# ElijahHyndman/PAPTeam_OpticalFlow

Measured on AMD Instinct MI355X. Metric: Mpix/s per frame-pair (fixed SOR iters) at 1920x1080; max-abs d(u,v) vs ref, higher is better.
Workload: dtype f64

## Files before the change

papteam_opticalflow_amd/csrc/kernels.hip:

```cpp
#include "common.h"
#include "sampler.h"

#include <cmath>

namespace papof {

namespace {

constexpr int BX = 64, BY = 4;

inline dim3 grid2d(int W, int H, int planes = 1) { return dim3((W + BX - 1) / BX, (H + BY - 1) / BY, planes); }
inline Rect region(const Rect* rc, int W, int H) { return rc ? *rc : Rect{0, 0, W, H}; }
inline dim3 grid2d(const Rect& r, int planes = 1) { return grid2d(r.x1 - r.x0, r.y1 - r.y0, planes); }

__device__ __forceinline__ void stamp_now(unsigned long long* s) {
    if (s && (blockIdx.x | blockIdx.y | blockIdx.z | threadIdx.x | threadIdx.y) == 0u) *s = __builtin_amdgcn_s_memrealtime();
}
__global__ void k_stamp(unsigned long long* s) { stamp_now(s); }

__device__ __forceinline__ int clampi(int x, int n) {
    x = x < 0 ? 0 : x;
    return x > n - 1 ? n - 1 : x;
}

__device__ __forceinline__ bool xcd_tile(int ntx, int nty, int& tx, int& ty) {
    const int ntiles = ntx * nty, per = (ntiles + 7) >> 3;
    const int vt = (int)(blockIdx.x & 7u) * per + (int)(blockIdx.x >> 3);
    if ((int)(blockIdx.x >> 3) >= per || vt >= ntiles) return false;
    ty = vt / ntx;
    tx = vt - ty * ntx;
    return true;
}
static inline unsigned xcd_grid(int ntx, int nty) { return 8u * (unsigned)(((size_t)ntx * nty + 7) / 8); }

__global__ void k_hwc_to_planar(const double* __restrict__ hwc, double* __restrict__ planar, int H, int W, int C) {
    const int j = blockIdx.x * BX + threadIdx.x, i = blockIdx.y * BY + threadIdx.y;
    if (j >= W || i >= H) return;
    const size_t o = (size_t)i * W + j, np = (size_t)H * W;
    hwc += blockIdx.z * np * C;
    planar += blockIdx.z * np * C;
    for (int k = 0; k < C; k++) planar[k * np + o] = hwc[o * C + k];
}

__global__ void k_hwc_u8_to_planar(const unsigned char* __restrict__ hwc, double* __restrict__ planar, int H, int W,
                                   int C) {
    const int j = blockIdx.x * BX + threadIdx.x, i = blockIdx.y * BY + threadIdx.y;
    if (j >= W || i >= H) return;
    const size_t o = (size_t)i * W + j, np = (size_t)H * W;
    hwc += blockIdx.z * np * C;
    planar += blockIdx.z * np * C;
    for (int k = 0; k < C; k++) planar[k * np + o] = (double)hwc[o * C + k] / 255.0;
}

__global__ void k_planar_to_hwc(const double* __restrict__ planar, double* __restrict__ hwc, int H, int W, int C) {
    const int j = blockIdx.x * BX + threadIdx.x, i = blockIdx.y * BY + threadIdx.y;
    if (j >= W || i >= H) return;
    const size_t o = (size_t)i * W + j, np = (size_t)H * W;
    for (int k = 0; k < C; k++) hwc[o * C + k] = planar[k * np + o];
}

__device__ __forceinline__ double tensor_load(const void* p, int dtype, long long o) {
    if (dtype == PAPOF_DTYPE_U8) return (double)static_cast<const unsigned char*>(p)[o] / 255.0;
    if (dtype == PAPOF_DTYPE_F32) return (double)static_cast<const float*>(p)[o];
    return static_cast<const double*>(p)[o];
}

__global__ __launch_bounds__(256) void k_ingest_frames(const papof_tensor a, const papof_tensor b, int pairs,
                                                       double* __restrict__ planar, long long H, long long W, long long C,
                                                       long long total) {
    const long long i = (long long)blockIdx.x * blockDim.x + threadIdx.x;
    if (i >= total) return;
    const long long np = H * W, f = i / (np * C), r = i - f * np * C, c = r / np, px = r - c * np, row = px / W,
                    col = px - row * W;
    const bool second = pairs && (f & 1);
    const long long fi = pairs ? f >> 1 : f;
    const long long o = fi * (second ? b.stride[0] : a.stride[0]) + row * (second ? b.stride[1] : a.stride[1]) +
                        col * (second ? b.stride[2] : a.stride[2]) + c * (second ? b.stride[3] : a.stride[3]);
    planar[i] = tensor_load(second ? b.data : a.data, second ? b.dtype : a.dtype, o);
}

constexpr double kInitMax = 1e6;
__device__ __forceinline__ bool init_refused(double x) { return !(fabs(x) <= kInitMax); }

__global__ __launch_bounds__(256) void k_init_check(const papof_tensor t, long long H, long long W, long long total,
                                                    unsigned* __restrict__ flag) {
    const long long i = (long long)blockIdx.x * blockDim.x + threadIdx.x;
    if (i >= total) return;
    const long long np = H * W, p = i / (np * 2), r = i - p * np * 2, c = r / np, px = r - c * np, row = px / W,
                    col = px - row * W;
    const long long o = p * t.stride[0] + row * t.stride[1] + col * t.stride[2] + c * t.stride[3];
    if (init_refused(tensor_load(t.data, t.dtype, o))) atomicOr(flag, 1u);
}

__global__ __launch_bounds__(256) void k_init_sanitize(double* __restrict__ planar, long long total) {
    const long long i = (long long)blockIdx.x * blockDim.x + threadIdx.x;
    if (i >= total) return;
    if (init_refused(planar[i])) planar[i] = 0.0;
}

__global__ __launch_bounds__(256) void k_emit_outputs(const double* __restrict__ src, const papof_tensor dst, int comp_major,
                                                      long long H, long long W, long long K, long long total) {
    const long long i = (long long)blockIdx.x * blockDim.x + threadIdx.x;
    if (i >= total) return;
    const long long np = H * W, p = i / (np * K), r = i - p * np * K;
    const long long k = comp_major ? r / np : r % K, px = comp_major ? r - k * np : r / K, row = px / W, col = px - row * W;
    const long long o = p * dst.stride[0] + row * dst.stride[1] + col * dst.stride[2] + k * dst.stride[3];
    const double v = src[i];
    if (dst.dtype == PAPOF_DTYPE_F32)
        static_cast<float*>(dst.data)[o] = (float)v;
    else
        static_cast<double*>(dst.data)[o] = v;
}

constexpr int kFbTX = 64, kFbTY = 4;
__global__ __launch_bounds__(kFbTX * kFbTY) void k_fb_check(const papof_tensor fw, const papof_tensor bw, const papof_tensor mask,
                                                         int H, int W, double a1, double a2) {
    const int tx = (W + kFbTX - 1) / kFbTX;
    const int x = (int)(blockIdx.x % tx) * kFbTX + threadIdx.x, r = (int)(blockIdx.x / tx) * kFbTY + threadIdx.y;
    if (x >= W || r >= H) return;
    const long long p = blockIdx.y >> 1;
    const int dir = blockIdx.y & 1;
    const papof_tensor& f = dir ? bw : fw;
    const papof_tensor& b = dir ? fw : bw;
    const long long of = p * f.stride[0] + r * f.stride[1] + x * f.stride[2];
    const double u = load_flow(f, of), v = load_flow(f, of + f.stride[3]);
    const double X = (double)x + u, Y = (double)r + v;
    bool occluded = true;
    if (X >= 0 && X <= (double)(W - 1) && Y >= 0 && Y <= (double)(H - 1)) {
        double bu, bv;
        sample_flow(b, p * b.stride[0], taps_at(X, Y, H, W), bu, bv);
        occluded = !fb_passes(u, v, bu, bv, a1, a2);
    }
    static_cast<unsigned char*>(mask.data)[p * mask.stride[0] + r * mask.stride[1] + x * mask.stride[2] + dir * mask.stride[3]] =
        occluded ? 1 : 0;
}

__global__ void k_filter_h(const double* __restrict__ src, double* __restrict__ dst, int H, int W, Taps f, Rect rc) {
    const int j = rc.x0 + blockIdx.x * BX + threadIdx.x, i = rc.y0 + blockIdx.y * BY + threadIdx.y;
    if (j >= rc.x1 || i >= rc.y1) return;
    const size_t np = (size_t)H * W;
    const double* row = src + blockIdx.z * np + (size_t)i * W;
    double acc = 0.0;
    for (int l = -f.fsize; l <= f.fsize; l++) acc += row[clampi(j + l, W)] * f.t[l + f.fsize];
    dst[blockIdx.z * np + (size_t)i * W + j] = acc;
}

__global__ void k_filter_v(const double* __restrict__ src, double* __restrict__ dst, int H, int W, Taps f, Rect rc) {
    const int j = rc.x0 + blockIdx.x * BX + threadIdx.x, i = rc.y0 + blockIdx.y * BY + threadIdx.y;
    if (j >= rc.x1 || i >= rc.y1) return;
    const size_t np = (size_t)H * W;
    const double* p = src + blockIdx.z * np + j;
    double acc = 0.0;
    for (int l = -f.fsize; l <= f.fsize; l++) acc += p[(size_t)clampi(i + l, H) * W] * f.t[l + f.fsize];
    dst[blockIdx.z * np + (size_t)i * W + j] = acc;
}

// ... 622 lines not shown
        } else if (I.lap != nullptr && I.lap[k] < 1E-20) {
            psi = 0.0;
        } else {
            psi = 1 / (2 * sqrt(t + 0.001 * 0.001));
        }
        const double pgx = psi * gx, pgy = psi * gy;
        if (planes == 1) {
            sxy = pgx * gy;
            sx2 = pgx * gx;
            sy2 = pgy * gy;
            stx = pgx * gt;
            sty = pgy * gt;
        } else {
            sxy += pgx * gy;
            sx2 += pgx * gx;
            sy2 += pgy * gy;
            stx += pgx * gt;
            sty += pgy * gt;
        }
    };
    if (PLANES > 0) {
#pragma unroll
        for (int k = 0; k < PLANES; k++) channel(k);
    } else {
#pragma unroll 1
        for (int k = 0; k < planes; k++) channel(k);
    }
    if (planes > 1) {
        sxy = sxy / planes;
        sx2 = sx2 / planes;
        sy2 = sy2 / planes;
        stx = stx / planes;
        sty = sty / planes;
    }
    SystemCell c;
    if (EDGE) {
        c.b1 = -stx - alpha * laplacian_at(u, phi, i, j, H, W);
        c.b2 = -sty - alpha * laplacian_at(v, phi, i, j, H, W);
        sor_diagonals(phi, i, j, H, W, sx2, sy2, alpha, omega, c.a1, c.a2);
    } else {
        const double pc = phi[o], pl = phi[o - 1], pu = phi[o - W];
        const double uc = u[o], vc = v[o];
        double lu = 0.0, lv = 0.0;
        lu -= (u[o + 1] - uc) * pc;
        lu += (uc - u[o - 1]) * pl;
        lu -= (u[o + W] - uc) * pc;
        lu += (uc - u[o - W]) * pu;
        lv -= (v[o + 1] - vc) * pc;
        lv += (vc - v[o - 1]) * pl;
        lv -= (v[o + W] - vc) * pc;
        lv += (vc - v[o - W]) * pu;
        c.b1 = -stx - alpha * lu;
        c.b2 = -sty - alpha * lv;
        double coeff = 0.0;
        coeff += pl;
        coeff += pc;
        coeff += pu;
        coeff += pc;
        coeff *= alpha;
        c.a1 = omega / (sx2 + alpha * 0.05 + coeff);
        c.a2 = omega / (sy2 + alpha * 0.05 + coeff);
    }
    c.phi = phi[o];
    c.xy = sxy;
    c.x2 = sx2;
    c.y2 = sy2;
    return c;
}

__global__ void k_assemble(const double* __restrict__ blend, const double* __restrict__ imdt,
                           const double* __restrict__ phi, const double* __restrict__ u,
                           const double* __restrict__ v, int H, int W, int planes, double alpha, double omega,
                           double* __restrict__ o_phi, double* __restrict__ o_xy, double* __restrict__ o_a1,
                           double* __restrict__ o_a2, double* __restrict__ o_b1, double* __restrict__ o_b2,
                           double* __restrict__ o_x2, double* __restrict__ o_y2, Taps d, Increment I, Rect rc,
                           unsigned long long* stamp) {
    stamp_now(stamp);
    const int j = rc.x0 + blockIdx.x * BX + threadIdx.x, i = rc.y0 + blockIdx.y * BY + threadIdx.y;
    if (j >= rc.x1 || i >= rc.y1) return;
    const size_t o = (size_t)i * W + j;
    const SystemCell c = assemble_cell(blend, imdt, phi, u, v, i, j, H, W, planes, alpha, omega, d, I);
    o_phi[o] = c.phi;
    o_xy[o] = c.xy;
    o_a1[o] = c.a1;
    o_a2[o] = c.a2;
    o_b1[o] = c.b1;
    o_b2[o] = c.b2;
    if (o_x2) o_x2[o] = c.x2;
    if (o_y2) o_y2[o] = c.y2;
}

#ifndef PAPOF_V_ASMCOLS
#define PAPOF_V_ASMCOLS 16
#endif
constexpr int kTileJ = PAPOF_V_ASMCOLS;
#ifndef PAPOF_V_ASMROWS
#define PAPOF_V_ASMROWS 16
#endif
constexpr int kAsmRows = PAPOF_V_ASMROWS;
struct double2s {
    double x, y;
};
template <int PLANES, bool FAST>
__global__ __launch_bounds__(256) void k_assemble_skew(const double* __restrict__ blend,
                                                       const double* __restrict__ imdt,
                                                       const double* __restrict__ phi, const double* __restrict__ u,
                                                       const double* __restrict__ v, int H, int W, int planes,
                                                       double alpha, double omega, SkewIdx sk,
                                                       double2s* __restrict__ pa, double2s* __restrict__ pb,
                                                       double2s* __restrict__ pc, double* __restrict__ o_x2,
                                                       double* __restrict__ o_y2, Taps d, Increment I,
                                                       unsigned long long* stamp, int row0, int row1) {
    __shared__ double stage[6][kAsmRows][kTileJ + 1];
    stamp_now(stamp);
    const int ib = row0 + blockIdx.y * kAsmRows, j0 = blockIdx.x * kTileJ, tid = threadIdx.x;
    const bool interior = ib >= 2 && ib + kAsmRows + 2 <= H && j0 >= 2 && j0 + kTileJ + 2 <= W;
    for (int c = tid; c < kAsmRows * kTileJ; c += 256) {
        const int r = c / kTileJ, jj = c - r * kTileJ;
        const int i = ib + r, j = j0 + jj;
        if (i < row1 && j < W) {
            const SystemCell s =
                interior ? assemble_cell<false, PLANES, FAST>(blend, imdt, phi, u, v, i, j, H, W, planes, alpha, omega, d, I)
                         : assemble_cell<true, PLANES, FAST>(blend, imdt, phi, u, v, i, j, H, W, planes, alpha, omega, d, I);
            stage[0][r][jj] = s.phi;
            stage[1][r][jj] = s.xy;
            stage[2][r][jj] = s.a1;
            stage[3][r][jj] = s.a2;
            stage[4][r][jj] = s.b1;
            stage[5][r][jj] = s.b2;
            if (o_x2) o_x2[(size_t)i * W + j] = s.x2;
            if (o_y2) o_y2[(size_t)i * W + j] = s.y2;
        }
    }
    __syncthreads();
    const int g = tid / kTileJ, jj = tid - g * kTileJ;
    const int j = j0 + jj;
    if (j >= W) return;
    for (int pp = g; pp <= kAsmRows + kTileJ - 2; pp += 256 / kTileJ) {
        const int r = pp - jj;
        if (r < 0 || r >= kAsmRows) continue;
        const int i = ib + r;
        if (i >= row1) continue;
        const size_t q = skew_cell(i, j, sk);
        pa[q] = double2s{stage[0][r][jj], stage[1][r][jj]};
        pb[q] = double2s{stage[2][r][jj], stage[3][r][jj]};
        pc[q] = double2s{stage[4][r][jj], stage[5][r][jj]};
    }
}

constexpr int kFT = 16, kFH = 4, kFW = kFT + 2 * kFH;
struct SixPlanes {
    double* q[6];
};
template <int PLANES, bool SKEW, bool BATCH = false>
__global__ __launch_bounds__(256, 1) void k_flow_system(const double* __restrict__ im1, const double* __restrict__ im2,
                                                     const double* __restrict__ u, const double* __restrict__ v,
                                                     const double* __restrict__ im1s, int H, int W, double alpha,
                                                     double omega, SkewIdx sk, SixPlanes out, Taps g, Taps d,
                                                     unsigned long long* stamp, unsigned* __restrict__ wit, double wit_thr,
                                                     unsigned mark, int row0, int row1, BatchK bk) {
    if (BATCH) {
        const size_t p = blockIdx.y;
        im1s += batch_frames(bk, p, im1, im2);
        u += p * bk.uv;
        v += p * bk.uv;
        if (wit != nullptr) wit += p * bk.wit;
#pragma unroll
        for (int q = 0; q < 6; q++) out.q[q] += p * bk.sp;
    }
    constexpr int NT = kFT * kFT, HWc = kFT + 2 * kFH;
    __shared__ double raw[kFW][HWc + 1];
    __shared__ double hs[kFW][kFT + 4 + 1];
    __shared__ double bl[kFT + 4][kFT + 4 + 1];
    __shared__ double it[kFT][kFT + 1];
    __shared__ double ph[kFT + 1][kFT + 1 + 1];
    __shared__ double stage[6][kFT][kFT + 1];
    stamp_now(stamp);
    const int ntx = (W + kFT - 1) / kFT, ntiles = ntx * ((row1 - row0 + kFT - 1) / kFT), per = (ntiles + 7) >> 3;
    const int vt = (int)(blockIdx.x & 7u) * per + (int)(blockIdx.x >> 3);
    if ((int)(blockIdx.x >> 3) >= per || vt >= ntiles) return;
    const int tby = vt / ntx, tbx = vt - tby * ntx;
    const int ib = row0 + tby * kFT, j0 = tbx * kFT, tid = threadIdx.x;
    const size_t np = (size_t)H * W;
    const int vy0 = max(0, row0 - kFH), vy1 = min(H, row1 + kFH);
    const bool interior = ib >= vy0 + kFH && ib + kFT <= row1 && ib + kFT + kFH <= vy1 && j0 >= kFH && j0 + kFT + kFH <= W;
    constexpr int kPer = (kFW * HWc + NT - 1) / NT;
    int t_o[kPer], t_x0[kPer], t_y0[kPer];
    double t_dx[kPer], t_dy[kPer];
    bool t_in[kPer], t_out[kPer];
#pragma unroll
    for (int q = 0; q < kPer; q++) {
        const int c = tid + q * NT, r = c / HWc, cc = c - r * HWc;
        const int i = ib - kFH + r, j = j0 - kFH + cc;
        t_in[q] = c < kFW * HWc && i >= vy0 && i < vy1 && j >= 0 && j < W;
        t_o[q] = t_in[q] ? i * W + j : 0;
        double x = 0.0, y = 0.0;
        t_out[q] = false;
        if (t_in[q]) {
            y = i + v[t_o[q]];
            x = j + u[t_o[q]];
            t_out[q] = x < 0 || x > W - 1 || y < 0 || y > H - 1;
            if (t_out[q]) {
                x = j;
                y = i;
            }
        }
        t_x0[q] = (int)x;
        t_y0[q] = (int)y;
        t_dx[q] = x - t_x0[q];
        t_dy[q] = y - t_y0[q];
    }
    for (int c = tid; c < (kFT + 1) * (kFT + 1); c += NT) {
        const int r = c / (kFT + 1), cc = c - r * (kFT + 1);
        const int i = ib - 1 + r, j = j0 - 1 + cc;
        if (i < 0 || i >= min(H, row1) || j < 0 || j >= W) continue;
        const size_t o = (size_t)i * W + j;
        const double uc = u[o], vc = v[o];
        double ur = 0.0, vr = 0.0, ud = 0.0, vd = 0.0;
        if (j < W - 1) {
            ur = u[o + 1];
            vr = v[o + 1];
        }
        if (i < H - 1) {
            ud = u[o + W];
            vd = v[o + W];
        }
        const double ux = j < W - 1 ? ur - uc : 0.0;
        const double uy = i < H - 1 ? ud - uc : 0.0;
        const double vx = j < W - 1 ? vr - vc : 0.0;
        const double vy = i < H - 1 ? vd - vc : 0.0;
        const double tt = ux * ux + uy * uy + vx * vx + vy * vy;
        ph[r][cc] = 0.5 / sqrt(tt + 0.001 * 0.001);
    }
    const int orow = tid / kFT, ocol = tid - orow * kFT;
    const int oi = ib + orow, oj = j0 + ocol;
    const bool own = oi < row1 && oj < W;
    double sxy = 0.0, sx2 = 0.0, sy2 = 0.0, stx = 0.0, sty = 0.0;
    const bool sampler = wit != nullptr && tid < 64 &&
                         (ntiles <= 256 || ((tbx + 5 * tby) & 15) == 0);
    constexpr int kP3 = ((kFT + 4) * (kFT + 4) + NT - 1) / NT;
    double gv[kPer][4], s1v[kP3], wv = 0.0;
    const auto load_gathers = [&](int k) {
        const double *p1 = im1 + k * np, *p2 = im2 + k * np;
#pragma unroll
        for (int q = 0; q < kPer; q++) {
            const double* src = t_out[q] ? p1 : p2;
            const int x0 = t_x0[q], y0 = t_y0[q], x1 = min(x0 + 1, W - 1), y1 = min(y0 + 1, H - 1);
            gv[q][0] = src[y0 * W + x0];
            gv[q][1] = src[y1 * W + x0];
            gv[q][2] = src[y0 * W + x1];
            gv[q][3] = src[y1 * W + x1];
        }
        if (sampler) wv = p1[t_o[0]];
    };
    const auto load_s1 = [&](int k) {
        const double* ps = im1s + k * np;
#pragma unroll
        for (int q = 0; q < kP3; q++) {
            const int c = min(tid + q * NT, (kFT + 4) * (kFT + 4) - 1), r = c / (kFT + 4), cc = c - r * (kFT + 4);
            s1v[q] = ps[(size_t)clampi(ib - 2 + r, H) * W + clampi(j0 - 2 + cc, W)];
        }
    };
    load_gathers(0);
    load_s1(0);
#pragma unroll 1
    for (int k = 0; k < PLANES; k++) {
        bool hit = false;
#pragma unroll
        for (int q = 0; q < kPer; q++) {
            const int c = tid + q * NT, r = c / HWc, cc = c - r * HWc;
            const double dx = t_dx[q], dy = t_dy[q], ex = 1.0 - dx, ey = 1.0 - dy;
            double res = 0.0;
            res += gv[q][0] * (ex * ey);
            res += gv[q][1] * (ex * dy);
            res += gv[q][2] * (dx * ey);
            res += gv[q][3] * (dx * dy);
            res = t_out[q] ? gv[q][0] : res;
            if (t_in[q]) raw[r][cc] = res;
            if (sampler && q == 0) {
                const double dd = fabs(wv - res);
                hit = t_in[q] && dd >= wit_thr && dd < 1000000;
            }
        }
        if (sampler) {
            const unsigned long long hits = __ballot(hit);
            if (hits != 0ull && tid == 0) wit[k] = mark;
        }
        if (k + 1 < PLANES) load_gathers(k + 1);
        __syncthreads();
        if (interior) {
            for (int c = tid; c < kFW * (kFT + 4); c += NT) {
                const int r = c / (kFT + 4), cc = c - r * (kFT + 4);
                double acc = 0.0;
#pragma unroll
                for (int l = -2; l <= 2; l++) acc += raw[r][cc + 2 + l] * g.t[l + 2];
                hs[r][cc] = acc;
            }
        } else {
            for (int c = tid; c < kFW * (kFT + 4); c += NT) {
                const int r = c / (kFT + 4), cc = c - r * (kFT + 4);
                const int i = ib - kFH + r, j = j0 - 2 + cc;
                if (i < 0 || i >= H || j < 0 || j >= W) continue;
                double acc = 0.0;
#pragma unroll
                for (int l = -2; l <= 2; l++) acc += raw[r][clampi(j + l, W) - (j0 - kFH)] * g.t[l + 2];
                hs[r][cc] = acc;
            }
        }
        __syncthreads();
#pragma unroll
        for (int q = 0; q < kP3; q++) {
            const int c = tid + q * NT, r = c / (kFT + 4), cc = c - r * (kFT + 4);
            const int i = ib - 2 + r, j = j0 - 2 + cc;
            if (c >= (kFT + 4) * (kFT + 4) || i < 0 || i >= H || j < 0 || j >= W) continue;
            double s2 = 0.0;
            if (interior) {
#pragma unroll
                for (int l = -2; l <= 2; l++) s2 += hs[r + 2 + l][cc] * g.t[l + 2];
            } else {
#pragma unroll
                for (int l = -2; l <= 2; l++) s2 += hs[clampi(i + l, H) - (ib - kFH)][cc] * g.t[l + 2];
            }
            const double s1 = s1v[q];
            double t = s1;
            t *= 0.4;
            t += s2 * 0.6;
            bl[r][cc] = t;
            if (r >= 2 && r < kFT + 2 && cc >= 2 && cc < kFT + 2) it[r - 2][cc - 2] = s2 - s1;
        }
        if (k + 1 < PLANES) load_s1(k + 1);
        __syncthreads();
        if (own) {
            double gx = 0.0, gy = 0.0;
            if (interior) {
#pragma unroll
                for (int l = -2; l <= 2; l++) gx += bl[orow + 2][ocol + 2 + l] * d.t[l + 2];
#pragma unroll
                for (int l = -2; l <= 2; l++) gy += bl[orow + 2 + l][ocol + 2] * d.t[l + 2];
            } else {
#pragma unroll
                for (int l = -2; l <= 2; l++) gx += bl[orow + 2][clampi(oj + l, W) - (j0 - 2)] * d.t[l + 2];
#pragma unroll
                for (int l = -2; l <= 2; l++) gy += bl[clampi(oi + l, H) - (ib - 2)][ocol + 2] * d.t[l + 2];
            }
            const double gt = it[orow][ocol];
            double t = gt;
            t *= t;
            const double psi = 1 / (2 * sqrt(t + 0.001 * 0.001));
            const double pgx = psi * gx, pgy = psi * gy;
            if (PLANES == 1) {
                sxy = pgx * gy;
                sx2 = pgx * gx;
                sy2 = pgy * gy;
                stx = pgx * gt;
                sty = pgy * gt;
            } else {
                sxy += pgx * gy;
                sx2 += pgx * gx;
                sy2 += pgy * gy;
                stx += pgx * gt;
                sty += pgy * gt;
            }
        }
    }
    if (own) {
        if (PLANES > 1) {
            sxy = sxy / PLANES;
            sx2 = sx2 / PLANES;
            sy2 = sy2 / PLANES;
            stx = stx / PLANES;
            sty = sty / PLANES;
        }
        const int i = oi, j = oj;
        const size_t o = (size_t)i * W + j;
        const double pc_ = ph[orow + 1][ocol + 1];
        const double pl = j > 0 ? ph[orow + 1][ocol] : 0.0, pu = i > 0 ? ph[orow][ocol + 1] : 0.0;
        const double uc = u[o], vc = v[o];
        double lu = 0.0, lv = 0.0;
        if (j < W - 1) {
            lu -= (u[o + 1] - uc) * pc_;
            if (j > 0) lu += (uc - u[o - 1]) * pl;
        }
        if (i < H - 1) {
            lu -= (u[o + W] - uc) * pc_;
            if (i > 0) lu += (uc - u[o - W]) * pu;
        }
        if (j < W - 1) {
            lv -= (v[o + 1] - vc) * pc_;
            if (j > 0) lv += (vc - v[o - 1]) * pl;
        }
        if (i < H - 1) {
            lv -= (v[o + W] - vc) * pc_;
            if (i > 0) lv += (vc - v[o - W]) * pu;
        }
        double coeff = 0.0;
        if (j > 0) coeff += pl;
        if (j < W - 1) coeff += pc_;
        if (i > 0) coeff += pu;
        if (i < H - 1) coeff += pc_;
        coeff *= alpha;
        const double a1 = omega / (sx2 + alpha * 0.05 + coeff), a2 = omega / (sy2 + alpha * 0.05 + coeff);
        const double b1 = -stx - alpha * lu, b2 = -sty - alpha * lv;
        if (SKEW) {
            stage[0][orow][ocol] = pc_;
            stage[1][orow][ocol] = sxy;
            stage[2][orow][ocol] = a1;
            stage[3][orow][ocol] = a2;
            stage[4][orow][ocol] = b1;
            stage[5][orow][ocol] = b2;
        } else {
            out.q[0][o] = pc_;
            out.q[1][o] = sxy;
            out.q[2][o] = a1;
            out.q[3][o] = a2;
            out.q[4][o] = b1;
            out.q[5][o] = b2;
        }
    }
    if (!SKEW) return;
    double2s* const pa = reinterpret_cast<double2s*>(out.q[0]);
    double2s* const pb = reinterpret_cast<double2s*>(out.q[2]);
    double2s* const pc = reinterpret_cast<double2s*>(out.q[4]);
    __syncthreads();
    const int grp = tid / kFT, jj = tid - grp * kFT, j = j0 + jj;
    if (j >= W) return;
    for (int pp = grp; pp <= 2 * kFT - 2; pp += kFT) {
        const int r = pp - jj;
        if (r < 0 || r >= kFT) continue;
        const int i = ib + r;
        if (i >= row1) continue;
        const size_t q = skew_cell(i, j, sk);
        pa[q] = double2s{stage[0][r][jj], stage[1][r][jj]};
        pb[q] = double2s{stage[2][r][jj], stage[3][r][jj]};
        pc[q] = double2s{stage[4][r][jj], stage[5][r][jj]};
    }
}

template <bool SKEW>
__global__ void k_sor_prep(const double* __restrict__ phi, const double* __restrict__ imdxy,
                           const double* __restrict__ imdx2, const double* __restrict__ imdy2,
                           const double* __restrict__ rhs1, const double* __restrict__ rhs2, int H, int W,
                           double alpha, double omega, SkewIdx sk, double* __restrict__ o_phi,
                           double* __restrict__ o_xy, double* __restrict__ o_a1, double* __restrict__ o_a2,
                           double* __restrict__ o_b1, double* __restrict__ o_b2) {
    const int j = blockIdx.x * BX + threadIdx.x, i = blockIdx.y * BY + threadIdx.y;
    if (j >= W || i >= H) return;
    const size_t o = (size_t)i * W + j;
    double a1, a2;
    sor_diagonals(phi, i, j, H, W, imdx2[o], imdy2[o], alpha, omega, a1, a2);
    const size_t q = sor_index<SKEW>(i, j, W, sk);
    o_phi[q] = phi[o];
    o_xy[q] = imdxy[o];
    o_a1[q] = a1;
    o_a2[q] = a2;
    o_b1[q] = rhs1[o];
    o_b2[q] = rhs2[o];
}

template <bool SKEW>
__global__ void k_sor_unpack(const double* __restrict__ sdu, const double* __restrict__ sdv,
                             double* __restrict__ du, double* __restrict__ dv, int H, int W, SkewIdx sk) {
    const int j = blockIdx.x * BX + threadIdx.x, i = blockIdx.y * BY + threadIdx.y;
    if (j >= W || i >= H) return;
    const size_t o = (size_t)i * W + j;
    if (SKEW) {
        const size_t q = 2 * dudv_cell(i, j, sk);
        du[o] = sdu[q];
        dv[o] = sdu[q + 1];
    } else {
        du[o] = sdu[o];
        dv[o] = sdv[o];
    }
}

__global__ void k_update_warp(const double* __restrict__ sdu, const double* __restrict__ sdv, double* __restrict__ u,
                              double* __restrict__ v, const double* __restrict__ im1,
                              const double* __restrict__ im2, double* __restrict__ warp, int H, int W, int planes, Rect rc,
                              int do_warp, unsigned long long* stamp) {
    stamp_now(stamp);
    const int j = rc.x0 + blockIdx.x * BX + threadIdx.x, i = rc.y0 + blockIdx.y * BY + threadIdx.y;
    if (j >= rc.x1 || i >= rc.y1) return;
// ... 414 lines not shown
}

int filter_hv(papof_handle* h, const double* src, double* dst, double* tmp, int H, int W, int planes, const Taps& fh,
              const Taps& fv) {
    if (fh.fsize > kHvMaxF || fv.fsize > kHvMaxF) {
        if (!tmp) return PAPOF_EINVAL;
        PAPOF_TRY(filter_h(h, src, tmp, H, W, planes, fh));
        return filter_v(h, tmp, dst, H, W, planes, fv);
    }
    const dim3 grid((W + BX - 1) / BX, (H + kHvRows - 1) / kHvRows, planes), block(BX, BY);
    const int f = fh.fsize == fv.fsize ? fh.fsize : -1;
    if (PAPOF_V_HVSTAGED && f >= 1 && f <= 3) {
        const dim3 sgrid(xcd_grid((W + BX - 1) / BX, (H + kHvsRows - 1) / kHvsRows), 1, planes);
        if (f == 1)
            hipLaunchKernelGGL(k_filter_hv_staged<1>, sgrid, block, 0, h->stream, src, dst, H, W, fh, fv);
        else if (f == 2)
            hipLaunchKernelGGL(k_filter_hv_staged<2>, sgrid, block, 0, h->stream, src, dst, H, W, fh, fv);
        else
            hipLaunchKernelGGL(k_filter_hv_staged<3>, sgrid, block, 0, h->stream, src, dst, H, W, fh, fv);
        LAUNCH_CHECK();
        return PAPOF_OK;
    }
    if (f == 1)
        hipLaunchKernelGGL(k_filter_hv<1>, grid, block, 0, h->stream, src, dst, H, W, fh, fv);
    else if (f == 2)
        hipLaunchKernelGGL(k_filter_hv<2>, grid, block, 0, h->stream, src, dst, H, W, fh, fv);
    else if (f == 3)
        hipLaunchKernelGGL(k_filter_hv<3>, grid, block, 0, h->stream, src, dst, H, W, fh, fv);
    else
        hipLaunchKernelGGL(k_filter_hv<-1>, grid, block, 0, h->stream, src, dst, H, W, fh, fv);
    LAUNCH_CHECK();
    return PAPOF_OK;
}

int resize(papof_handle* h, const double* src, double* dst, int sh, int sw, int planes, int dh, int dw, double xr,
           double yr, bool use_post, double post, const Rect* rc) {
    const Rect r = region(rc, dw, dh);
    if (r.empty()) return PAPOF_OK;
    hipLaunchKernelGGL(k_resize, dim3(xcd_grid((r.x1 - r.x0 + BX - 1) / BX, (r.y1 - r.y0 + BY - 1) / BY), 1, planes), dim3(BX, BY), 0, h->stream, src, dst, sh, sw, dh, dw, xr, yr,
                       use_post ? 1 : 0, post, r, take_stamp(h));
    LAUNCH_CHECK();
    return PAPOF_OK;
}

int im2feature(papof_handle* h, const double* im, double* feat, int H, int W, int C, unsigned* nz, int frames, size_t nz_stride) {
    const size_t np = (size_t)H * W;
    if (C == 3) {
        hipLaunchKernelGGL((frames > 1 ? k_im2feature_tiled<3, true> : k_im2feature_tiled<3, false>), dim3(xcd_grid((W + BX - 1) / BX, (H + kFeatRows - 1) / kFeatRows), frames), dim3(BX, BY), 0,
                           h->stream, im, feat, H, W, deriv5_taps(), nz, h->lap_epoch, 3 * np, 5 * np, nz_stride);
    } else if (C == 1) {
        hipLaunchKernelGGL((frames > 1 ? k_im2feature_tiled<1, true> : k_im2feature_tiled<1, false>), dim3(xcd_grid((W + BX - 1) / BX, (H + kFeatRows - 1) / kFeatRows), frames), dim3(BX, BY), 0,
                           h->stream, im, feat, H, W, deriv5_taps(), nz, h->lap_epoch, np, 3 * np, nz_stride);
    } else {
        if (frames != 1) return PAPOF_EINVAL;
        PAPOF_HIP(hipMemcpyAsync(feat, im, sizeof(double) * (size_t)H * W * C, hipMemcpyDeviceToDevice, h->stream));
        return PAPOF_OK;
    }
    LAUNCH_CHECK();
    return PAPOF_OK;
}

int warp_bilinear(papof_handle* h, const double* im1, const double* im2, const double* vx, const double* vy,
                  double* out, int H, int W, int planes, const Rect* rc) {
    const Rect r = region(rc, W, H);
    if (r.empty()) return PAPOF_OK;
    hipLaunchKernelGGL(k_warp, grid2d(r), dim3(BX, BY), 0, h->stream, im1, im2, vx, vy, out, H, W, planes, r,
                       take_stamp(h));
    LAUNCH_CHECK();
    return PAPOF_OK;
}

int smooth_v_blend(papof_handle* h, const double* tmp, const double* im1s, double* blend, double* imdt, int H,
                   int W, int planes, const Rect* rc) {
    const Rect r = region(rc, W, H);
    if (r.empty()) return PAPOF_OK;
    hipLaunchKernelGGL(k_smooth_v_blend, grid2d(r, planes), dim3(BX, BY), 0, h->stream, tmp, im1s, blend, imdt, H, W,
                       smooth5_taps(), r);
    LAUNCH_CHECK();
    return PAPOF_OK;
}

static SkewIdx skew_idx(const SorPlanes& sp) {
    return SkewIdx{sp.sd.hp, sp.sd.qt, sp.sd.rt, sp.sd.nb, sp.sd.npos_d, sp.sd.dpar, sp.sd.band_rows, sp.sd.koff, sp.sd.poff};
}

static Increment increment_of(const SorPlanes* prev, const double* gm = nullptr, const double* lap = nullptr) {
    if (!prev) return Increment{nullptr, nullptr, 0, SkewIdx{0, 0, 0, 0, 0, 0, 0}, gm, lap};
    return Increment{prev->du, prev->dv, prev->skew ? 1 : 0, prev->skew ? skew_idx(*prev) : SkewIdx{0, 0, 0, 0, 0, 0, 0},
                     gm, lap};
}

int smooth_hv_blend(papof_handle* h, const double* warp, const double* im1s, double* blend, double* imdt, int H,
                    int W, int planes, int row0, int row1) {
    if (row1 < 0) row1 = H;
    if (row0 < 0 || row1 > H) return PAPOF_EINVAL;
    if (row1 <= row0) return PAPOF_OK;
    hipLaunchKernelGGL(k_smooth_hv_blend, dim3((W + BX - 1) / BX, (row1 - row0 + kFuseRows - 1) / kFuseRows, planes),
                       dim3(BX, BY), 0, h->stream, warp, im1s, blend, imdt, H, W, smooth5_taps(), take_stamp(h), row0,
                       row1);
    LAUNCH_CHECK();
    return PAPOF_OK;
}

int warp_smooth_blend(papof_handle* h, const double* im1, const double* im2, const double* u, const double* v,
                      const double* im1s, double* blend, double* imdt, int H, int W, int planes, unsigned* wit,
                      double* phi_out) {
    hipLaunchKernelGGL(k_warp_smooth_blend, dim3((W + BX - 1) / BX, (H + kWsRows - 1) / kWsRows, planes), dim3(BX, BY), 0,
                       h->stream, im1, im2, u, v, im1s, blend, imdt, H, W, smooth5_taps(), take_stamp(h), wit,
                       2e-20 * (double)H * (double)W, h->lap_epoch, phi_out);
    LAUNCH_CHECK();
    return PAPOF_OK;
}

int compute_phi(papof_handle* h, const double* u, const double* v, const SorPlanes* prev, double* phi, int H, int W,
                const Rect* rc) {
    const Rect r = region(rc, W, H);
    if (r.empty()) return PAPOF_OK;
    hipLaunchKernelGGL(k_phi, grid2d(r), dim3(BX, BY), 0, h->stream, u, v, increment_of(prev), phi, H, W, r,
                       take_stamp(h));
    LAUNCH_CHECK();
    return PAPOF_OK;
}

int assemble_system(papof_handle* h, const double* blend, const double* imdt, const double* phi, const double* u,
                    const double* v, int H, int W, int planes, double alpha, double omega, const SorPlanes& out,
                    double* opt_imdx2, double* opt_imdy2, const SorPlanes* prev, const Rect* rc, const double* gm,
                    const double* lap) {
    const Increment I = increment_of(prev, gm, lap);
    const Rect r = region(rc, W, H);
    if (r.empty()) return PAPOF_OK;
    if (out.skew) {
        if (rc && (r.x0 != 0 || r.x1 != W)) return PAPOF_EINVAL;
        const bool fast = I.du == nullptr && I.gm == nullptr && I.lap == nullptr;
        const auto kern = planes == 5   ? (fast ? k_assemble_skew<5, true> : k_assemble_skew<5, false>)
                          : planes == 3 ? (fast ? k_assemble_skew<3, true> : k_assemble_skew<3, false>)
                                        : k_assemble_skew<0, false>;
        hipLaunchKernelGGL(kern, dim3((W + kTileJ - 1) / kTileJ, (r.y1 - r.y0 + kAsmRows - 1) / kAsmRows),
                           dim3(256), 0, h->stream, blend, imdt, phi, u, v, H, W, planes, alpha, omega, skew_idx(out),
                           (double2s*)out.phi, (double2s*)out.a1, (double2s*)out.b1, opt_imdx2, opt_imdy2,
                           deriv5_taps(), I, take_stamp(h), r.y0, r.y1);
    } else {
        hipLaunchKernelGGL(k_assemble, grid2d(r), dim3(BX, BY), 0, h->stream, blend, imdt, phi, u, v, H, W, planes,
                           alpha, omega, out.phi, out.xy, out.a1, out.a2, out.b1, out.b2, opt_imdx2, opt_imdy2,
                           deriv5_taps(), I, r, take_stamp(h));
    }
    LAUNCH_CHECK();
    return PAPOF_OK;
}

int flow_system(papof_handle* h, const double* im1, const double* im2, const double* u, const double* v, const double* im1s,
                int H, int W, int planes, double alpha, double omega, const SorPlanes& out, unsigned* wit, int row0, int row1,
                int batch, const BatchK* bk) {
    if (planes != 5 && planes != 3) return PAPOF_EINVAL;
    if (row1 < 0) row1 = H;
    if (row0 < 0 || row1 > H) return PAPOF_EINVAL;
    if (row1 <= row0) return PAPOF_OK;
    const int ntiles = ((W + kFT - 1) / kFT) * ((row1 - row0 + kFT - 1) / kFT);
    const dim3 grid(8 * ((ntiles + 7) / 8), batch);
    const SixPlanes six{{out.phi, out.xy, out.a1, out.a2, out.b1, out.b2}};
    const BatchK bk0{0, 0, 0, 0, 0, 0};
    const auto kern = batch > 1 ? (out.skew ? (planes == 5 ? k_flow_system<5, true, true> : k_flow_system<3, true, true>)
                                            : (planes == 5 ? k_flow_system<5, false, true> : k_flow_system<3, false, true>))
                                : (out.skew ? (planes == 5 ? k_flow_system<5, true> : k_flow_system<3, true>)
                                            : (planes == 5 ? k_flow_system<5, false> : k_flow_system<3, false>));
    hipLaunchKernelGGL(kern, grid, dim3(kFT * kFT), 0, h->stream, im1, im2, u, v, im1s, H, W, alpha, omega,
                       out.skew ? skew_idx(out) : SkewIdx{0, 0, 0, 0, 0, 0, 0, 0, 0}, six, smooth5_taps(), deriv5_taps(),
                       take_stamp(h), wit, 2e-20 * (double)H * (double)W, h->lap_epoch, row0, row1, bk ? *bk : bk0);
    LAUNCH_CHECK();
    return PAPOF_OK;
}

int laplacian(papof_handle* h, const double* in, const double* weight, double* out, int H, int W) {
    hipLaunchKernelGGL(k_laplacian, grid2d(W, H), dim3(BX, BY), 0, h->stream, in, weight, out, H, W);
    LAUNCH_CHECK();
    return PAPOF_OK;
}

int update_and_warp(papof_handle* h, const SorPlanes& sp, double* u, double* v, const double* im1,
                    const double* im2, double* warp, int H, int W, int planes, bool do_warp) {
    if (sp.skew) {
        hipLaunchKernelGGL(k_update_warp_skew, grid2d(W, H), dim3(BX, BY), 0, h->stream, (const double2s*)sp.du, u, v,
                           im1, im2, warp, H, W, planes, skew_idx(sp), take_stamp(h), do_warp ? 1 : 0);
    } else {
        hipLaunchKernelGGL(k_update_warp, grid2d(W, H), dim3(BX, BY), 0, h->stream, sp.du, sp.dv, u, v, im1, im2, warp,
                           H, W, planes, Rect{0, 0, W, H}, do_warp ? 1 : 0, take_stamp(h));
    }
    LAUNCH_CHECK();
    return PAPOF_OK;
}

int update_warp_phi(papof_handle* h, const SorPlanes& sp, const double* u, const double* v, double* u_out, double* v_out,
                    const double* im1, const double* im2, double* warp, double* phi_out, int H, int W, int planes,
                    bool do_warp, int row0, int row1, unsigned* wit, int batch, const BatchK* bk) {
    const double wit_thr = 2e-20 * (double)H * (double)W;
    const BatchK bk0{0, 0, 0, 0, 0, 0};
    if (batch > 1 && (warp || phi_out || do_warp)) return PAPOF_EINVAL;
    if (u == u_out || v == v_out) return PAPOF_EINVAL;
    if (row1 < 0) row1 = H;
    if (row0 < 0 || row1 > H) return PAPOF_EINVAL;
    if (row1 <= row0) return PAPOF_OK;
    const dim3 grid(xcd_grid((W + BX - 1) / BX, (row1 - row0 + BY - 1) / BY), batch);
    if (sp.skew)
        hipLaunchKernelGGL((batch > 1 ? k_update_warp_phi<true, true> : k_update_warp_phi<true, false>), grid, dim3(BX, BY), 0,
                           h->stream, sp.du, sp.dv, skew_idx(sp),
                           u, v, u_out, v_out, im1, im2, warp, phi_out, H, W, planes, do_warp ? 1 : 0, take_stamp(h),
                           row0, row1, wit, wit_thr, h->lap_epoch, bk ? *bk : bk0);
    else
        hipLaunchKernelGGL((batch > 1 ? k_update_warp_phi<false, true> : k_update_warp_phi<false, false>), grid, dim3(BX, BY), 0, h->stream, sp.du, sp.dv,
                           SkewIdx{0, 0, 0, 0, 0, 0, 0, 0, 0}, u, v, u_out, v_out, im1, im2, warp, phi_out, H, W, planes,
                           do_warp ? 1 : 0, take_stamp(h), row0, row1, wit, wit_thr, h->lap_epoch, bk ? *bk : bk0);
    LAUNCH_CHECK();
    return PAPOF_OK;
}

int update_flow(papof_handle* h, const SorPlanes& sp, double* u, double* v, int H, int W, const Rect& r) {
    if (sp.skew) return PAPOF_EINVAL;
    if (r.empty()) return PAPOF_OK;
    hipLaunchKernelGGL(k_update_warp, grid2d(r), dim3(BX, BY), 0, h->stream, sp.du, sp.dv, u, v, nullptr, nullptr, nullptr,
                       H, W, 0, r, 0, take_stamp(h));
    LAUNCH_CHECK();
    return PAPOF_OK;
}

int flow_quantize16(papof_handle* h, const double* vx, const double* vy, unsigned short* q, size_t n) {
    if (!n) return PAPOF_OK;
    hipLaunchKernelGGL(k_flow_quantize16, dim3((unsigned)((n + 255) / 256)), dim3(256), 0, h->stream, vx, vy, q, n);
    LAUNCH_CHECK();
    return PAPOF_OK;
}

int flow_dequantize16(papof_handle* h, const unsigned short* q, double* vx, double* vy, size_t n) {
    if (!n) return PAPOF_OK;
    hipLaunchKernelGGL(k_flow_dequantize16, dim3((unsigned)((n + 255) / 256)), dim3(256), 0, h->stream, q, vx, vy, n);
    LAUNCH_CHECK();
    return PAPOF_OK;
}

int flow_to_bgr(papof_handle* h, const double* vx, const double* vy, size_t n, double* partial ,
                unsigned char* bgr) {
    if (!n) return PAPOF_OK;
    const int nblocks = 256;
    hipLaunchKernelGGL(k_flow_mag_minmax, dim3(nblocks), dim3(256), 0, h->stream, vx, vy, n, partial);
    hipLaunchKernelGGL(k_flow_bgr, dim3((unsigned)((n + 255) / 256)), dim3(256), 0, h->stream, vx, vy, n, partial,
                       nblocks, bgr);
    LAUNCH_CHECK();
    return PAPOF_OK;
}

int bicubic_warp(papof_handle* h, const double* im1, const double* im2, const double* gx, const double* gy,
                 const double* gxy, const double* vx, const double* vy, double* out_hwc, int H, int W, int C,
                 const Rect* rc, bool planar_out, bool clamp, int batch, const BatchK* bk) {
    const Rect r = region(rc, W, H);
    if (r.empty()) return PAPOF_OK;
    const BatchK bk0{0, 0, 0, 0, 0, 0};
    hipLaunchKernelGGL(batch > 1 ? k_bicubic<true> : k_bicubic<false>, dim3(xcd_grid((r.x1 - r.x0 + BX - 1) / BX, (r.y1 - r.y0 + BY - 1) / BY), batch), dim3(BX, BY), 0, h->stream, im1, im2, gx, gy, gxy, vx, vy, out_hwc, H, W,
                       C, r, take_stamp(h), planar_out ? 1 : 0, clamp ? 1 : 0, bk ? *bk : bk0);
    LAUNCH_CHECK();
    return PAPOF_OK;
}

constexpr int kGmBlocks = 256, kGmThreads = 256, kGmMaxC = 8;
static __global__ __launch_bounds__(kGmThreads) void k_gm_partial(const double* __restrict__ im1,
                                                           const double* __restrict__ im2, size_t np, int C,
                                                           const double* __restrict__ gm, double* __restrict__ partial) {
    __shared__ double red[kGmThreads];
    double acc[kGmMaxC][4];
    for (int k = 0; k < kGmMaxC; k++) acc[k][0] = acc[k][1] = acc[k][2] = acc[k][3] = 0.0;
    for (size_t o = (size_t)blockIdx.x * kGmThreads + threadIdx.x; o < np; o += (size_t)kGmBlocks * kGmThreads) {
#pragma unroll
        for (int k = 0; k < kGmMaxC; k++) {
            if (k >= C) break;
            double t = im1[k * np + o] - im2[k * np + o];
            t *= t;
            const double alpha_k = gm[k], sigma = gm[C + k], beta = gm[2 * C + k], s2 = gm[3 * C + k], b2 = gm[4 * C + k];
            double w1 = exp(-t / (2 * s2)) / (2 * 3.1415927 * sigma) * alpha_k;
            double w2 = exp(-t / (2 * b2)) / (2 * 3.1415927 * beta) * (1 - alpha_k);
            const double s = w1 + w2;
            w1 /= s;
            w2 /= s;
            acc[k][0] += w1;
            acc[k][1] += w2;
            acc[k][2] += w1 * t;
            acc[k][3] += w2 * t;
        }
    }
    for (int k = 0; k < C; k++)
        for (int q = 0; q < 4; q++) {
            red[threadIdx.x] = acc[k][q];
            __syncthreads();
            for (int s = kGmThreads / 2; s > 0; s >>= 1) {
                if ((int)threadIdx.x < s) red[threadIdx.x] += red[threadIdx.x + s];
                __syncthreads();
            }
            if (threadIdx.x == 0) partial[((size_t)blockIdx.x * kGmMaxC + k) * 4 + q] = red[0];
            __syncthreads();
        }
}

static __global__ void k_gm_mstep(const double* __restrict__ partial, int C, double prior, double* __restrict__ gm) {
    const int k = threadIdx.x;
    if (k >= C) return;
    double t1 = 0.0, t2 = 0.0, s1 = 0.05, s2 = 0.5;
    for (int b = 0; b < kGmBlocks; b++) {
        const double* p = partial + ((size_t)b * kGmMaxC + k) * 4;
        t1 += p[0];
        t2 += p[1];
        s1 += p[2];
        s2 += p[3];
    }
    const double alpha = t1 / (t1 + t2) * (1 - prior) + 0.95 * prior;
    const double sigma = sqrt(s1 / t1);
    const double beta = sqrt(s2 / t2) * (1 - prior) + 0.3 * prior;
    gm[k] = alpha;
    gm[C + k] = sigma;
    gm[2 * C + k] = beta;
    gm[3 * C + k] = sigma * sigma;
    gm[4 * C + k] = beta * beta;
// ... 168 lines not shown
```

Before: 210.0.

## Vectorize warp gathers, precompute byte offsets, and compute two blur outputs per thread

```diff
diff --git a/papteam_opticalflow_amd/csrc/kernels.hip b/papteam_opticalflow_amd/csrc/kernels.hip
--- a/papteam_opticalflow_amd/csrc/kernels.hip
+++ b/papteam_opticalflow_amd/csrc/kernels.hip
@@ -2,6 +2,7 @@
 #include "sampler.h"
 
 #include <cmath>
+#include <type_traits>
 
 namespace papof {
 
@@ -930,7 +931,14 @@
 struct SixPlanes {
     double* q[6];
 };
-template <int PLANES, bool SKEW, bool BATCH = false>
+typedef double tap_pair __attribute__((ext_vector_type(2), aligned(8)));
+__device__ __forceinline__ double plane_ld(const double* plane, unsigned byte_off) {
+    return *reinterpret_cast<const double*>(reinterpret_cast<const char*>(plane) + byte_off);
+}
+__device__ __forceinline__ tap_pair plane_ld2(const double* plane, unsigned byte_off) {
+    return *reinterpret_cast<const tap_pair*>(reinterpret_cast<const char*>(plane) + byte_off);
+}
+template <int PLANES, bool SKEW, bool BATCH = false, bool W1 = false>
 __global__ __launch_bounds__(256, 1) void k_flow_system(const double* __restrict__ im1, const double* __restrict__ im2,
                                                      const double* __restrict__ u, const double* __restrict__ v,
                                                      const double* __restrict__ im1s, int H, int W, double alpha,
@@ -963,31 +971,62 @@
     const int vy0 = max(0, row0 - kFH), vy1 = min(H, row1 + kFH);
     const bool interior = ib >= vy0 + kFH && ib + kFT <= row1 && ib + kFT + kFH <= vy1 && j0 >= kFH && j0 + kFT + kFH <= W;
     constexpr int kPer = (kFW * HWc + NT - 1) / NT;
-    int t_o[kPer], t_x0[kPer], t_y0[kPer];
+    static_assert(kFW * HWc == 2 * NT + 64 && NT + 16 < kFW * HWc, "the three slots of the warp");
+    const int lane = tid & 63, wave = __builtin_amdgcn_readfirstlane(tid >> 6);
+    constexpr bool w1 = W1;
+    unsigned t_o[kPer], t_b0[kPer], t_b1[kPer];
+    int t_ra[kPer];
     double t_dx[kPer], t_dy[kPer];
-    bool t_in[kPer], t_out[kPer];
-#pragma unroll
-    for (int q = 0; q < kPer; q++) {
-        const int c = tid + q * NT, r = c / HWc, cc = c - r * HWc;
-        const int i = ib - kFH + r, j = j0 - kFH + cc;
-        t_in[q] = c < kFW * HWc && i >= vy0 && i < vy1 && j >= 0 && j < W;
-        t_o[q] = t_in[q] ? i * W + j : 0;
-        double x = 0.0, y = 0.0;
-        t_out[q] = false;
-        if (t_in[q]) {
-            y = i + v[t_o[q]];
-            x = j + u[t_o[q]];
-            t_out[q] = x < 0 || x > W - 1 || y < 0 || y > H - 1;
-            if (t_out[q]) {
-                x = j;
-                y = i;
+    bool t_in[kPer], t_out[kPer], t_hi[kPer];
+    {
+        int r = tid / HWc, cc = tid - r * HWc;
+#pragma unroll
+        for (int q = 0; q < kPer; q++) {
+            if (q == 1) {
+                cc += NT - 10 * HWc;
+                r += 10;
+                if (cc >= HWc) {
+                    cc -= HWc;
+                    r++;
+                }
+            } else if (q == 2) {
+                cc = lane + (2 * NT - (2 * NT / HWc) * HWc);
+                r = 2 * NT / HWc;
+                if (cc >= HWc) {
+                    cc -= HWc;
+                    r++;
+                }
+                if (cc >= HWc) {
+                    cc -= HWc;
+                    r++;
+                }
             }
-        }
-        t_x0[q] = (int)x;
-        t_y0[q] = (int)y;
-        t_dx[q] = x - t_x0[q];
-        t_dy[q] = y - t_y0[q];
-    }
+            const int i = ib - kFH + r, j = j0 - kFH + cc;
+            t_ra[q] = r * (HWc + 1) + cc;
+            t_in[q] = i >= vy0 && i < vy1 && j >= 0 && j < W;
+            const int o = t_in[q] ? i * W + j : 0;
+            t_o[q] = (unsigned)o * 8u;
+            double x = 0.0, y = 0.0;
+            t_out[q] = false;
+            if (t_in[q]) {
+                y = i + v[o];
+                x = j + u[o];
+                t_out[q] = x < 0 || x > W - 1 || y < 0 || y > H - 1;
+                if (t_out[q]) {
+                    x = j;
+                    y = i;
+                }
+            }
+            const int x0 = (int)x, y0 = (int)y, y1 = min(y0 + 1, H - 1);
+            const int xb = w1 ? 0 : min(x0, W - 2);
+            t_hi[q] = x0 == W - 1;
+            t_b0[q] = (unsigned)(y0 * W + xb) * 8u;
+            t_b1[q] = (unsigned)(y1 * W + xb) * 8u;
+            t_dx[q] = x - x0;
+            t_dy[q] = y - y0;
+        }
+    }
+    const bool wout = __ballot(t_out[0] || t_out[1] || t_out[2]) != 0ull;
     for (int c = tid; c < (kFT + 1) * (kFT + 1); c += NT) {
         const int r = c / (kFT + 1), cc = c - r * (kFT + 1);
         const int i = ib - 1 + r, j = j0 - 1 + cc;
@@ -1017,44 +1056,71 @@
     const bool sampler = wit != nullptr && tid < 64 &&
                          (ntiles <= 256 || ((tbx + 5 * tby) & 15) == 0);
     constexpr int kP3 = ((kFT + 4) * (kFT + 4) + NT - 1) / NT;
-    double gv[kPer][4], s1v[kP3], wv = 0.0;
+    int s_r[kP3], s_c[kP3];
+    unsigned s_o[kP3];
+    static_assert(kP3 == 2 && kFW * (kFT + 4) / 2 <= NT && (kFT + 4) * (kFT + 4) / 2 <= NT, "two outputs per thread");
+    const int h_r = tid / ((kFT + 4) / 2), h_c = 2 * (tid - h_r * ((kFT + 4) / 2));
+    {
+        const int t = min(tid, (kFT + 4) * (kFT + 4) / 2 - 1), rp = t / (kFT + 4);
+        s_r[0] = 2 * rp;
+        s_r[1] = 2 * rp + 1;
+        s_c[0] = s_c[1] = t - rp * (kFT + 4);
+    }
+#pragma unroll
+    for (int q = 0; q < kP3; q++)
+        s_o[q] = (unsigned)(clampi(ib - 2 + s_r[q], H) * W + clampi(j0 - 2 + s_c[q], W)) * 8u;
+    double* const rawf = &raw[0][0];
+    tap_pair ga[kPer], gb[kPer];
+    double f1v[kPer] = {0.0, 0.0, 0.0}, s1v[kP3], wv = 0.0;
     const auto load_gathers = [&](int k) {
         const double *p1 = im1 + k * np, *p2 = im2 + k * np;
+        const bool third = (k & 3) == wave;
 #pragma unroll
         for (int q = 0; q < kPer; q++) {
-            const double* src = t_out[q] ? p1 : p2;
-            const int x0 = t_x0[q], y0 = t_y0[q], x1 = min(x0 + 1, W - 1), y1 = min(y0 + 1, H - 1);
-            gv[q][0] = src[y0 * W + x0];
-            gv[q][1] = src[y1 * W + x0];
-            gv[q][2] = src[y0 * W + x1];
-            gv[q][3] = src[y1 * W + x1];
-        }
-        if (sampler) wv = p1[t_o[0]];
+            if (q == 2 && !third) continue;
+            if (w1) {
+                ga[q].x = plane_ld(p2, t_b0[q]);
+                gb[q].x = plane_ld(p2, t_b1[q]);
+            } else {
+                ga[q] = plane_ld2(p2, t_b0[q]);
+                gb[q] = plane_ld2(p2, t_b1[q]);
+            }
+            if (wout) f1v[q] = plane_ld(p1, t_o[q]);
+        }
+        if (sampler) wv = plane_ld(p1, t_o[0]);
     };
     const auto load_s1 = [&](int k) {
         const double* ps = im1s + k * np;
 #pragma unroll
-        for (int q = 0; q < kP3; q++) {
-            const int c = min(tid + q * NT, (kFT + 4) * (kFT + 4) - 1), r = c / (kFT + 4), cc = c - r * (kFT + 4);
-            s1v[q] = ps[(size_t)clampi(ib - 2 + r, H) * W + clampi(j0 - 2 + cc, W)];
-        }
+        for (int q = 0; q < kP3; q++) s1v[q] = plane_ld(ps, s_o[q]);
+    };
+    const auto two_sums = [&](const double(&x)[6], double& a0, double& a1) {
+        a0 = 0.0;
+        a1 = 0.0;
+#pragma unroll
+        for (int l = 0; l < 5; l++) a0 += x[l] * g.t[l];
+#pragma unroll
+        for (int l = 0; l < 5; l++) a1 += x[l + 1] * g.t[l];
     };
     load_gathers(0);
     load_s1(0);
 #pragma unroll 1
     for (int k = 0; k < PLANES; k++) {
         bool hit = false;
+        const bool third = (k & 3) == wave;
 #pragma unroll
         for (int q = 0; q < kPer; q++) {
-            const int c = tid + q * NT, r = c / HWc, cc = c - r * HWc;
+            if (q == 2 && !third) continue;
             const double dx = t_dx[q], dy = t_dy[q], ex = 1.0 - dx, ey = 1.0 - dy;
+            const double g0 = !w1 && t_hi[q] ? ga[q].y : ga[q].x, g1 = !w1 && t_hi[q] ? gb[q].y : gb[q].x;
+            const double g2 = w1 ? ga[q].x : ga[q].y, g3 = w1 ? gb[q].x : gb[q].y;
             double res = 0.0;
-            res += gv[q][0] * (ex * ey);
-            res += gv[q][1] * (ex * dy);
-            res += gv[q][2] * (dx * ey);
-            res += gv[q][3] * (dx * dy);
-            res = t_out[q] ? gv[q][0] : res;
-            if (t_in[q]) raw[r][cc] = res;
+            res += g0 * (ex * ey);
+            res += g1 * (ex * dy);
+            res += g2 * (dx * ey);
+            res += g3 * (dx * dy);
+            res = t_out[q] ? f1v[q] : res;
+            if (t_in[q]) rawf[t_ra[q]] = res;
             if (sampler && q == 0) {
                 const double dd = fabs(wv - res);
                 hit = t_in[q] && dd >= wit_thr && dd < 1000000;
@@ -1066,45 +1132,53 @@
         }
         if (k + 1 < PLANES) load_gathers(k + 1);
         __syncthreads();
-        if (interior) {
-            for (int c = tid; c < kFW * (kFT + 4); c += NT) {
-                const int r = c / (kFT + 4), cc = c - r * (kFT + 4);
-                double acc = 0.0;
-#pragma unroll
-                for (int l = -2; l <= 2; l++) acc += raw[r][cc + 2 + l] * g.t[l + 2];
-                hs[r][cc] = acc;
+        if (tid < kFW * (kFT + 4) / 2) {
+            const double* const row = raw[h_r];
+            double x[6], a0, a1;
+            if (interior) {
+#pragma unroll
+                for (int m = 0; m < 6; m++) x[m] = row[h_c + m];
+                two_sums(x, a0, a1);
+                hs[h_r][h_c] = a0;
+                hs[h_r][h_c + 1] = a1;
+            } else {
+                const int i = ib - kFH + h_r, j = j0 - 2 + h_c;
+                const bool ok0 = j >= 0 && j < W, ok1 = j + 1 >= 0 && j + 1 < W;
+                if (i >= 0 && i < H && (ok0 || ok1)) {
+#pragma unroll
+                    for (int m = 0; m < 6; m++) x[m] = row[clampi(j - 2 + m, W) - (j0 - kFH)];
+                    two_sums(x, a0, a1);
+                    if (ok0) hs[h_r][h_c] = a0;
+                    if (ok1) hs[h_r][h_c + 1] = a1;
+                }
             }
-        } else {
-            for (int c = tid; c < kFW * (kFT + 4); c += NT) {
-                const int r = c / (kFT + 4), cc = c - r * (kFT + 4);
-                const int i = ib - kFH + r, j = j0 - 2 + cc;
-                if (i < 0 || i >= H || j < 0 || j >= W) continue;
-                double acc = 0.0;
-#pragma unroll
-                for (int l = -2; l <= 2; l++) acc += raw[r][clampi(j + l, W) - (j0 - kFH)] * g.t[l + 2];
-                hs[r][cc] = acc;
+        }
+        __syncthreads();
+        if (tid < (kFT + 4) * (kFT + 4) / 2) {
+            const int r0 = s_r[0], cc = s_c[0], i = ib - 2 + r0, j = j0 - 2 + cc;
+            const bool okj = j >= 0 && j < W, ok0 = okj && i >= 0 && i < H, ok1 = okj && i + 1 >= 0 && i + 1 < H;
+            if (ok0 || ok1) {
+                double x[6], a[2];
+                if (interior) {
+#pragma unroll
+                    for (int m = 0; m < 6; m++) x[m] = hs[r0 + m][cc];
+                } else {
+#pragma unroll
+                    for (int m = 0; m < 6; m++) x[m] = hs[clampi(i - 2 + m, H) - (ib - kFH)][cc];
+                }
+                two_sums(x, a[0], a[1]);
+#pragma unroll
+                for (int e = 0; e < 2; e++) {
+                    if (!(e ? ok1 : ok0)) continue;
+                    const int r = r0 + e;
+                    const double s2 = a[e], s1 = s1v[e];
+                    double t = s1;
+                    t *= 0.4;
+                    t += s2 * 0.6;
+                    bl[r][cc] = t;
+                    if (r >= 2 && r < kFT + 2 && cc >= 2 && cc < kFT + 2) it[r - 2][cc - 2] = s2 - s1;
+                }
             }
-        }
-        __syncthreads();
-#pragma unroll
-        for (int q = 0; q < kP3; q++) {
-            const int c = tid + q * NT, r = c / (kFT + 4), cc = c - r * (kFT + 4);
-            const int i = ib - 2 + r, j = j0 - 2 + cc;
-            if (c >= (kFT + 4) * (kFT + 4) || i < 0 || i >= H || j < 0 || j >= W) continue;
-            double s2 = 0.0;
-            if (interior) {
-#pragma unroll
-                for (int l = -2; l <= 2; l++) s2 += hs[r + 2 + l][cc] * g.t[l + 2];
-            } else {
-#pragma unroll
-                for (int l = -2; l <= 2; l++) s2 += hs[clampi(i + l, H) - (ib - kFH)][cc] * g.t[l + 2];
-            }
-            const double s1 = s1v[q];
-            double t = s1;
-            t *= 0.4;
-            t += s2 * 0.6;
-            bl[r][cc] = t;
-            if (r >= 2 && r < kFT + 2 && cc >= 2 && cc < kFT + 2) it[r - 2][cc - 2] = s2 - s1;
         }
         if (k + 1 < PLANES) load_s1(k + 1);
         __syncthreads();
@@ -1825,6 +1899,7 @@
                 int H, int W, int planes, double alpha, double omega, const SorPlanes& out, unsigned* wit, int row0, int row1,
                 int batch, const BatchK* bk) {
     if (planes != 5 && planes != 3) return PAPOF_EINVAL;
+    if ((unsigned long long)H * (unsigned long long)W > (1ull << 29)) return PAPOF_EINVAL;
     if (row1 < 0) row1 = H;
     if (row0 < 0 || row1 > H) return PAPOF_EINVAL;
     if (row1 <= row0) return PAPOF_OK;
@@ -1832,10 +1907,14 @@
     const dim3 grid(8 * ((ntiles + 7) / 8), batch);
     const SixPlanes six{{out.phi, out.xy, out.a1, out.a2, out.b1, out.b2}};
     const BatchK bk0{0, 0, 0, 0, 0, 0};
-    const auto kern = batch > 1 ? (out.skew ? (planes == 5 ? k_flow_system<5, true, true> : k_flow_system<3, true, true>)
-                                            : (planes == 5 ? k_flow_system<5, false, true> : k_flow_system<3, false, true>))
-                                : (out.skew ? (planes == 5 ? k_flow_system<5, true> : k_flow_system<3, true>)
-                                            : (planes == 5 ? k_flow_system<5, false> : k_flow_system<3, false>));
+    const auto pick = [&](auto one_column) {
+        constexpr bool W1 = decltype(one_column)::value;
+        return batch > 1 ? (out.skew ? (planes == 5 ? k_flow_system<5, true, true, W1> : k_flow_system<3, true, true, W1>)
+                                     : (planes == 5 ? k_flow_system<5, false, true, W1> : k_flow_system<3, false, true, W1>))
+                         : (out.skew ? (planes == 5 ? k_flow_system<5, true, false, W1> : k_flow_system<3, true, false, W1>)
+                                     : (planes == 5 ? k_flow_system<5, false, false, W1> : k_flow_system<3, false, false, W1>));
+    };
+    const auto kern = W == 1 ? pick(std::true_type{}) : pick(std::false_type{});
     hipLaunchKernelGGL(kern, grid, dim3(kFT * kFT), 0, h->stream, im1, im2, u, v, im1s, H, W, alpha, omega,
                        out.skew ? skew_idx(out) : SkewIdx{0, 0, 0, 0, 0, 0, 0, 0, 0}, six, smooth5_taps(), deriv5_taps(),
                        take_stamp(h), wit, 2e-20 * (double)H * (double)W, h->lap_epoch, row0, row1, bk ? *bk : bk0);
```

Result: faster. 212.6 (median of 6 runs) (+1.2%).
